# KwonGihyun/TweedieMix

Measured on AMD Instinct MI355X. Metric: denoise steps/sec @ SDXL 1024^2 K=3 concepts (fusion phase); images/sec at 1/2/4/8 GPUs, higher is better.
Workload: dtype bf16

## Files before the change

tweediemix_amd/csrc/norm_misc.hip:

```cpp
#include "common.h"

namespace {

typedef __attribute__((ext_vector_type(8))) __bf16 frag_ab;

__device__ __forceinline__ void unpack8(const uint4& v, float (&f)[8]) {
    f[0] = bf2f((bf16_t)(v.x & 0xffff)); f[1] = bf2f((bf16_t)(v.x >> 16));
    f[2] = bf2f((bf16_t)(v.y & 0xffff)); f[3] = bf2f((bf16_t)(v.y >> 16));
    f[4] = bf2f((bf16_t)(v.z & 0xffff)); f[5] = bf2f((bf16_t)(v.z >> 16));
    f[6] = bf2f((bf16_t)(v.w & 0xffff)); f[7] = bf2f((bf16_t)(v.w >> 16));
}
__device__ __forceinline__ uint4 pack8(const float (&f)[8]) {
    uint4 v;
    v.x = pack_bf2(f[0], f[1]); v.y = pack_bf2(f[2], f[3]); v.z = pack_bf2(f[4], f[5]); v.w = pack_bf2(f[6], f[7]);
    return v;
}

constexpr int GN_MAX_C = 4096;

#ifndef GN_T
#define GN_T 128
#endif
#ifndef GN_APPLY_U
#define GN_APPLY_U 2
#endif
#ifndef GN_APPLY_ITEMS
#define GN_APPLY_ITEMS 1024
#endif
#ifndef GN_APPLY_MAXB
#define GN_APPLY_MAXB 4096
#endif
__host__ __device__ inline int gn_chunks(int64_t HW) {
    int64_t c = HW / 8;
    if (c > GN_T) c = GN_T;
    if (c < 1) c = 1;
    return (int)c;
}

__global__ void __launch_bounds__(256) gn_stats_kernel(const bf16_t* __restrict__ X1, int C1, const bf16_t* __restrict__ X2, int C2,
                                                       float* __restrict__ ws, int64_t HW, int groups, int chunks,
                                                       unsigned long long* prof) {
    __shared__ float s_sum[GN_MAX_C], s_sq[GN_MAX_C];
    if (prof && threadIdx.x == 0) prof_enter(prof, (blockIdx.x | blockIdx.y) == 0, 0);
    const int C = C1 + C2, nvec = C >> 3, cpg = C / groups;
    const int b = blockIdx.y, ch = blockIdx.x, tid = threadIdx.x;
    const int64_t ppc = (HW + chunks - 1) / chunks;
    const int64_t p0 = (int64_t)ch * ppc;
    int64_t p1 = p0 + ppc; if (p1 > HW) p1 = HW;
    const int plane = nvec <= 256 ? 256 / nvec : 1;
    for (int v0 = 0; v0 < nvec; v0 += 256) {
        const int v = v0 + (nvec <= 256 ? tid % nvec : tid);
        const int pl = nvec <= 256 ? tid / nvec : 0;
        if (v < nvec && pl < plane) {
            float a[8] = {0, 0, 0, 0, 0, 0, 0, 0}, q[8] = {0, 0, 0, 0, 0, 0, 0, 0};
            const int c0 = v * 8;
            const bf16_t* src; int cs, cl;
            if (c0 < C1) { src = X1 + (int64_t)b * HW * C1; cs = C1; cl = c0; }
            else         { src = X2 + (int64_t)b * HW * C2; cs = C2; cl = c0 - C1; }
            int64_t p = p0 + pl;
            for (; p + 3 * plane < p1; p += 4 * plane) {
                uint4 raw[4];
#pragma unroll
                for (int u = 0; u < 4; ++u) raw[u] = *(const uint4*)(src + (p + u * plane) * cs + cl);
#pragma unroll
                for (int u = 0; u < 4; ++u) {
                    float f[8]; unpack8(raw[u], f);
#pragma unroll
                    for (int j = 0; j < 8; ++j) { a[j] += f[j]; q[j] += f[j] * f[j]; }
                }
            }
            for (; p < p1; p += plane) {
                const uint4 raw = *(const uint4*)(src + p * cs + cl);
                float f[8]; unpack8(raw, f);
#pragma unroll
                for (int j = 0; j < 8; ++j) { a[j] += f[j]; q[j] += f[j] * f[j]; }
            }
#pragma unroll
            for (int j = 0; j < 8; ++j) { s_sum[pl * C + c0 + j] = a[j]; s_sq[pl * C + c0 + j] = q[j]; }
        }
    }
    __syncthreads();
    if (tid < groups) {
        float s = 0.f, q = 0.f;
// ... 39 lines not shown
        s += (a0 + a1) + (a2 + a3); q += (b0 + b1) + (b2 + b3);
    }
    for (; blk < nblk; blk += J, row += step) { s += row[0]; q += row[Cs]; }
}
__global__ void __launch_bounds__(GN_CS_T) gn_finalize_cs_kernel(const float* __restrict__ cs1, int C1, const float* __restrict__ cs2, int C2,
                                                                 const float* __restrict__ gamma, const float* __restrict__ beta,
                                                                 float2* __restrict__ ss, int64_t HW, int groups, float eps,
                                                                 unsigned long long* prof) {
    __shared__ double s_red[2 * GN_CS_T / 64];
    __shared__ float s_ms[2];
    if (prof && threadIdx.x == 0) prof_enter(prof, (blockIdx.x | blockIdx.y) == 0, 0);
    const int C = C1 + C2, cpg = C / groups;
    const int g = blockIdx.x, b = blockIdx.y, tid = threadIdx.x;
    const int nblk = (int)(HW / 32);
    float gm = 0.f, bt = 0.f;
    if (tid < cpg) { gm = gamma[g * cpg + tid]; bt = beta[g * cpg + tid]; }
    const int c_lo = g * cpg, c_hi = c_lo + cpg;
    const int n1 = min(c_hi, C1) - min(c_lo, C1), n2 = cpg - n1;
    float s = 0.f, q = 0.f;
    gn_cs_walk(cs1 + (int64_t)b * nblk * 2 * C1 + c_lo, C1, n1, nblk, tid, s, q);
    if (n2 > 0) gn_cs_walk(cs2 + (int64_t)b * nblk * 2 * C2 + (max(c_lo, C1) - C1), C2, n2, nblk, tid, s, q);
    double sd = (double)s, qd = (double)q;
#pragma unroll
    for (int o = 32; o > 0; o >>= 1) { sd += __shfl_xor(sd, o); qd += __shfl_xor(qd, o); }
    if ((tid & 63) == 0) { s_red[(tid >> 6) * 2] = sd; s_red[(tid >> 6) * 2 + 1] = qd; }
    __syncthreads();
    if (tid == 0) {
        double st = 0.0, qt = 0.0;
#pragma unroll
        for (int w = 0; w < GN_CS_T / 64; ++w) { st += s_red[2 * w]; qt += s_red[2 * w + 1]; }
        const double n = (double)HW * cpg;
        const double mean = st / n;
        double var = qt / n - mean * mean; if (var < 0.0) var = 0.0;
        s_ms[0] = (float)mean; s_ms[1] = (float)(1.0 / sqrt(var + (double)eps));
    }
    __syncthreads();
    if (tid < cpg) {
        const float sc = s_ms[1] * gm;
        ss[(int64_t)b * C + c_lo + tid] = make_float2(sc, bt - s_ms[0] * sc);
    }
}

__device__ __forceinline__ float silu_fast(float x) {
    return x * __builtin_amdgcn_rcpf(1.0f + __builtin_amdgcn_exp2f(-1.4426950408889634f * x));
}

__device__ __forceinline__ float gn_quad_max(float x) {
    float y = __int_as_float(__builtin_amdgcn_update_dpp(0, __float_as_int(x), 0xB1, 0xf, 0xf, false));
    x = fmaxf(x, y);
    y = __int_as_float(__builtin_amdgcn_update_dpp(0, __float_as_int(x), 0x4E, 0xf, 0xf, false));
    return fmaxf(x, y);
}

template <int F8>
__global__ void __launch_bounds__(256) gn_apply_kernel(const bf16_t* __restrict__ X1, int C1, const bf16_t* __restrict__ X2, int C2,
                                                       bf16_t* __restrict__ Y, const float2* __restrict__ ss, int64_t HW, int silu,
                                                       unsigned long long* prof, unsigned char* __restrict__ Y8 = nullptr, unsigned char* __restrict__ S8 = nullptr) {
    __shared__ float2 s_ss[GN_MAX_C];
    const unsigned long long pt0 = (prof && threadIdx.x == 0) ? prof_now() : 0;
    const int C = C1 + C2, nvec = C >> 3;
    const int b = blockIdx.y, tid = threadIdx.x;
    for (int c = tid; c < C; c += 256) s_ss[c] = ss[(int64_t)b * C + c];
    __syncthreads();
    const int64_t total = HW * nvec;
    int64_t per = (total + gridDim.x - 1) / gridDim.x;
    if (F8) per = (per + 3) & ~(int64_t)3;
    const int64_t i0 = (int64_t)blockIdx.x * per;
    int64_t i1 = i0 + per; if (i1 > total) i1 = total;
    int64_t p = i0 / nvec; int v = (int)(i0 - p * nvec) + tid;
    while (v >= nvec) { v -= nvec; ++p; }
    const int step_p = 256 / nvec, step_v = 256 - step_p * nvec;
    constexpr int U = GN_APPLY_U;
    for (int64_t i = i0 + tid; i < i1; i += 256 * U) {
        uint4 raw[U]; int64_t pp[U]; int cc[U];
#pragma unroll
        for (int u = 0; u < U; ++u) {
            pp[u] = p; cc[u] = v * 8;
            if (i + u * 256 < i1) {
                const bf16_t* src = (cc[u] < C1) ? X1 + ((int64_t)b * HW + p) * C1 + cc[u] : X2 + ((int64_t)b * HW + p) * C2 + (cc[u] - C1);
                raw[u] = *(const uint4*)src;
            }
            p += step_p; v += step_v;
            if (v >= nvec) { v -= nvec; ++p; }
        }
#pragma unroll
        for (int u = 0; u < U; ++u) {
            if (i + u * 256 < i1) {
                float f[8]; unpack8(raw[u], f);
#pragma unroll
                for (int j = 0; j < 8; ++j) {
                    const float2 k = s_ss[cc[u] + j];
                    float y = f[j] * k.x + k.y;
                    if (silu) y = silu_fast(y);
                    f[j] = y;
                }
                if constexpr (F8) {
                    const uint4 pk = pack8(f);
                    unpack8(pk, f);
                    float am = 0.f;
#pragma unroll
                    for (int j = 0; j < 8; ++j) am = fmaxf(am, fabsf(f[j]));
                    am = gn_quad_max(am);
                    const int e = e8m0_for_amax(am);
                    const float inv = exp2_neg_int(e);
                    int q0 = __builtin_amdgcn_cvt_pk_fp8_f32(f[0] * inv, f[1] * inv, 0, false); q0 = __builtin_amdgcn_cvt_pk_fp8_f32(f[2] * inv, f[3] * inv, q0, true);
                    int q1 = __builtin_amdgcn_cvt_pk_fp8_f32(f[4] * inv, f[5] * inv, 0, false); q1 = __builtin_amdgcn_cvt_pk_fp8_f32(f[6] * inv, f[7] * inv, q1, true);
                    const int64_t row = (int64_t)b * HW + pp[u];
                    *(uint2*)(Y8 + row * C + cc[u]) = make_uint2((unsigned)q0, (unsigned)q1);
                    if ((tid & 3) == 0) S8[row * (C >> 5) + (cc[u] >> 5)] = (unsigned char)(e + 127);
                } else
                *(uint4*)(Y + ((int64_t)b * HW + pp[u]) * C + cc[u]) = pack8(f);
            }
        }
    }
    if (prof && threadIdx.x == 0) prof_leave(prof, 0, pt0, pt0, pt0);
}

constexpr int GN_SMALL_MAX_CW = 256, GN_SMALL_MAX_ELEMS = 65536;
__global__ void __launch_bounds__(256) gn_small_kernel(const bf16_t* __restrict__ X1, int C1, const bf16_t* __restrict__ X2, int C2, bf16_t* __restrict__ Y,
                                                       const float* __restrict__ gamma, const float* __restrict__ beta, int HW, int groups, int gpw, float eps, int silu,
                                                       unsigned long long* prof) {
    __shared__ float r_s[2048], r_q[2048];
    __shared__ double c_s[GN_SMALL_MAX_CW], c_q[GN_SMALL_MAX_CW];
    __shared__ float g_ms[16];
    __shared__ float2 s_ss[GN_SMALL_MAX_CW];
    const unsigned long long pt0 = (prof && threadIdx.x == 0) ? prof_enter(prof, (blockIdx.x | blockIdx.y) == 0, 0) : 0;
    const int C = C1 + C2, cpg = C / groups, cw = gpw * cpg, nv = cw >> 3, rs = 256 / nv;
    const int b = blockIdx.y, c0 = blockIdx.x * cw, tid = threadIdx.x;
    const int v = tid % nv, slot = tid / nv;
    const bool active = slot < rs;
    const int cg = c0 + v * 8;
    const bf16_t* src; int ld;
    if (cg < C1) { src = X1 + (int64_t)b * HW * C1 + cg; ld = C1; } else { src = X2 + (int64_t)b * HW * C2 + (cg - C1); ld = C2; }
    float s[8], q[8];
#pragma unroll
    for (int j = 0; j < 8; ++j) { s[j] = 0.f; q[j] = 0.f; }
    if (active) {
        int row = slot;
        for (; row + 3 * rs < HW; row += 4 * rs) {
            uint4 raw[4];
#pragma unroll
            for (int u = 0; u < 4; ++u) raw[u] = *(const uint4*)(src + (int64_t)(row + u * rs) * ld);
#pragma unroll
            for (int u = 0; u < 4; ++u) {
                float f[8]; unpack8(raw[u], f);
#pragma unroll
                for (int j = 0; j < 8; ++j) { s[j] += f[j]; q[j] += f[j] * f[j]; }
            }
        }
        for (; row < HW; row += rs) {
            float f[8]; unpack8(*(const uint4*)(src + (int64_t)row * ld), f);
#pragma unroll
            for (int j = 0; j < 8; ++j) { s[j] += f[j]; q[j] += f[j] * f[j]; }
        }
#pragma unroll
        for (int j = 0; j < 8; ++j) { r_s[slot * cw + v * 8 + j] = s[j]; r_q[slot * cw + v * 8 + j] = q[j]; }
    }
    __syncthreads();
    if (tid < cw) {
        double a = 0.0, d = 0.0;
        for (int k = 0; k < rs; ++k) { a += (double)r_s[k * cw + tid]; d += (double)r_q[k * cw + tid]; }
        c_s[tid] = a; c_q[tid] = d;
    }
    __syncthreads();
    if (tid < gpw) {
        double a = 0.0, d = 0.0;
        for (int k = 0; k < cpg; ++k) { a += c_s[tid * cpg + k]; d += c_q[tid * cpg + k]; }
        const double n = (double)HW * cpg, mean = a / n;
// ... 177 lines not shown
                                                           const int* __restrict__ secs, int nsec, int Mtot, int mrow0) {
    const int lane = threadIdx.x & 63;
    const int n = blockIdx.x * 4 + (threadIdx.x >> 6);
    if (n >= N) return;
    float acc[MAXM];
#pragma unroll
    for (int m = 0; m < MAXM; ++m) acc[m] = 0.f;
    const int nvec = K >> 3;
    for (int v = lane; v < nvec; v += 64) {
        const uint4 raw = *(const uint4*)(W + (int64_t)n * K + v * 8);
        float wf[8]; unpack8(raw, wf);
#pragma unroll
        for (int m = 0; m < MAXM; ++m) {
            if (m < M) {
                const float4 x0 = *(const float4*)(in + (int64_t)m * K + v * 8);
                const float4 x1 = *(const float4*)(in + (int64_t)m * K + v * 8 + 4);
                float xf[8] = {x0.x, x0.y, x0.z, x0.w, x1.x, x1.y, x1.z, x1.w};
                if (act_in) {
#pragma unroll
                    for (int j = 0; j < 8; ++j) xf[j] = silu_f(xf[j]);
                }
#pragma unroll
                for (int j = 0; j < 8; ++j) acc[m] += xf[j] * wf[j];
            }
        }
    }
#pragma unroll
    for (int m = 0; m < MAXM; ++m) {
#pragma unroll
        for (int o = 32; o > 0; o >>= 1) acc[m] += __shfl_xor(acc[m], o);
    }
    if (lane == 0) {
        int64_t base = 0; int ldn = N, col = n;
        if (secs) {
            int sidx = 0;
            while (sidx + 1 < nsec && secs[sidx + 1] <= n) ++sidx;
            base = (int64_t)secs[sidx] * Mtot; ldn = secs[sidx + 1] - secs[sidx]; col = n - secs[sidx];
        }
        for (int m = 0; m < M; ++m) {
            float y = acc[m] + (bias ? bias[n] : 0.f) + (add ? add[(int64_t)m * N + n] : 0.f);
            if (act_out) y = silu_f(y);
            out[base + (int64_t)(secs ? mrow0 + m : m) * ldn + col] = y;
        }
    }
}

struct PreMap { float w[16]; float b[4]; int on; };

template <int CIN>
__global__ void __launch_bounds__(256) conv_in_kernel(const float* __restrict__ x, const float* __restrict__ w,
                                                      const float* __restrict__ bias, bf16_t* __restrict__ y,
                                                      int B, int H, int W, int Cout, const PreMap pm) {
    extern __shared__ __attribute__((aligned(16))) float s_w[];
    constexpr int KK = 9 * CIN;
    const int tid = threadIdx.x, lane = tid & 63;
    const int q = __builtin_amdgcn_readfirstlane(tid >> 6);
    for (int i = tid; i < Cout * KK / 4; i += 256) ((float4*)s_w)[i] = ((const float4*)w)[i];
    __syncthreads();
    const int64_t npix = (int64_t)B * H * W;
    for (int64_t tile = blockIdx.x; tile * 64 < npix; tile += gridDim.x) {
    int64_t pix = tile * 64 + lane;
    const bool live = pix < npix;
    if (!live) pix = npix - 1;
    const int b = (int)(pix / ((int64_t)H * W)); const int rem = (int)(pix - (int64_t)b * H * W);
    const int oy = rem / W, ox = rem - oy * W;
    float patch[KK];
#pragma unroll
    for (int ky = 0; ky < 3; ++ky)
#pragma unroll
        for (int kx = 0; kx < 3; ++kx) {
            const int iy = oy + ky - 1, ix = ox + kx - 1;
            const bool ok = iy >= 0 && iy < H && ix >= 0 && ix < W;
            float v[CIN];
#pragma unroll
            for (int ci = 0; ci < CIN; ++ci) v[ci] = ok ? x[(((int64_t)b * CIN + ci) * H + iy) * W + ix] : 0.f;
            if (pm.on && CIN == 4) {
                float u[4];
#pragma unroll
                for (int co = 0; co < 4; ++co)
                    u[co] = ok ? pm.b[co] + pm.w[co * 4 + 0] * v[0] + pm.w[co * 4 + 1] * v[1] + pm.w[co * 4 + 2] * v[2] + pm.w[co * 4 + 3] * v[3] : 0.f;
#pragma unroll
                for (int co = 0; co < 4; ++co) v[co] = u[co];
            }
#pragma unroll
            for (int ci = 0; ci < CIN; ++ci) patch[(ky * 3 + kx) * CIN + ci] = v[ci];
        }
    const int cpq = Cout / 4;
    for (int c0 = q * cpq; c0 < (q + 1) * cpq; c0 += 8) {
        float o[8];
#pragma unroll 2
        for (int j = 0; j < 8; ++j) {
            const float* wr = s_w + (c0 + j) * KK;
            float a = bias ? bias[c0 + j] : 0.f;
#pragma unroll
            for (int k = 0; k < KK; ++k) a += patch[k] * wr[k];
            o[j] = a;
        }
        if (live) *(uint4*)(y + pix * Cout + c0) = pack8(o);
    }
    }
}

__global__ void __launch_bounds__(256) conv_out_kernel(const bf16_t* __restrict__ x, const bf16_t* __restrict__ w,
                                                       const float* __restrict__ bias, float* __restrict__ y,
                                                       int B, int H, int W, int Cin, int Cout) {
    const int lane = threadIdx.x & 63, fr = lane & 15, fg = lane >> 4;
    const int64_t npix = (int64_t)B * H * W;
    const int64_t pbase = ((int64_t)blockIdx.x * 4 + (threadIdx.x >> 6)) * 16;
    if (pbase >= npix) return;
    int64_t pix = pbase + fr; if (pix > npix - 1) pix = npix - 1;
    const int b = (int)(pix / ((int64_t)H * W)); const int rem = (int)(pix - (int64_t)b * H * W);
    const int oy = rem / W, ox = rem - oy * W;
    const int co = fr < Cout ? fr : Cout - 1;
    const bf16_t* wrow = w + (int64_t)co * 9 * Cin;
    f32x4 acc = {0.f, 0.f, 0.f, 0.f};
    const frag_ab zero = {0, 0, 0, 0, 0, 0, 0, 0};
    for (int tap = 0; tap < 9; ++tap) {
        const int ky = tap / 3, kx = tap - ky * 3;
        const int iy = oy + ky - 1, ix = ox + kx - 1;
        const bool ok = iy >= 0 && iy < H && ix >= 0 && ix < W;
        const bf16_t* src = x + (((int64_t)b * H + (ok ? iy : 0)) * W + (ok ? ix : 0)) * Cin;
        for (int c = 0; c < Cin; c += 32) {
            frag_ab a = *(const frag_ab*)(src + c + fg * 8);
            if (!ok) a = zero;
            const frag_ab wf = *(const frag_ab*)(wrow + tap * Cin + c + fg * 8);
            acc = __builtin_amdgcn_mfma_f32_16x16x32_bf16(a, wf, acc, 0, 0, 0);
        }
    }
    if (fr < Cout) {
        const float bv = bias ? bias[fr] : 0.f;
#pragma unroll
        for (int r = 0; r < 4; ++r) {
            const int64_t pp = pbase + fg * 4 + r;
            if (pp < npix) {
                const int bb = (int)(pp / ((int64_t)H * W)); const int64_t rr = pp - (int64_t)bb * H * W;
                y[((int64_t)bb * Cout + fr) * H * W + rr] = acc[r] + bv;
            }
        }
    }
}

}

extern "C" int tmix_groupnorm_ws_chunks(int64_t HW) { return gn_chunks(HW); }
extern "C" int64_t tmix_groupnorm_ws_floats(int B, int C, int groups) { return (int64_t)B * GN_T * groups * 2 + (int64_t)B * C * 2; }

extern "C" int tmix_groupnorm_nhwc_launches(int64_t HW, int C, int groups) {
    if (HW <= 0 || C <= 0 || groups <= 0 || (C % groups)) return 0;
    return gn_small_gpw(HW, C, groups) ? 1 : 3;
}

extern "C" int tmix_groupnorm_nhwc(const void* X1, int C1, const void* X2, int C2, void* Y, const float* gamma,
                                   const float* beta, float* ws, int B, int64_t HW, int groups, float eps, int silu,
                                   void* stream) {
    if (!X1 || !Y || !gamma || !beta || !ws) TMIX_FAIL(TMIX_EINVAL, "groupnorm: null pointer");
    if (C2 > 0 && !X2) TMIX_FAIL(TMIX_EINVAL, "groupnorm: C2 > 0 but X2 is null");
    const int C = C1 + C2;
    if (B <= 0 || HW <= 0 || C <= 0) TMIX_FAIL(TMIX_ESHAPE, "groupnorm: empty problem");
    if ((C1 % 8) || (C2 % 8) || C > GN_MAX_C || groups <= 0 || groups > 64 || (C % groups)) TMIX_FAIL(TMIX_ESHAPE, "groupnorm: C1=%d C2=%d groups=%d unsupported", C1, C2, groups);
    if (!aligned16(X1) || (X2 && !aligned16(X2)) || !aligned16(Y)) TMIX_FAIL(TMIX_EALIGN, "groupnorm: pointers must be 16-byte aligned");
    const int chunks = gn_chunks(HW);
    hipStream_t st = (hipStream_t)stream;
    unsigned long long* prof = tmix_prof_take();
    if (const int gpw = gn_small_gpw(HW, C, groups)) {
        gn_small_kernel<<<dim3(groups / gpw, B), 256, 0, st>>>((const bf16_t*)X1, C1, (const bf16_t*)X2, C2, (bf16_t*)Y, gamma, beta, (int)HW, groups, gpw, eps, silu, prof);
        TMIX_LAUNCH_CHECK();
        return TMIX_OK;
    }
    gn_stats_kernel<<<dim3(chunks, B), 256, 0, st>>>((const bf16_t*)X1, C1, (const bf16_t*)X2, C2, ws, HW, groups, chunks, prof);
    TMIX_LAUNCH_CHECK();
    float2* ss = (float2*)(ws + (int64_t)B * GN_T * groups * 2);
    gn_finalize_kernel<<<dim3(groups, B), 64, 0, st>>>(ws, gamma, beta, ss, C, HW, groups, chunks, eps);
    TMIX_LAUNCH_CHECK();
    int64_t nb = (HW * (C / 8) + GN_APPLY_ITEMS - 1) / GN_APPLY_ITEMS; if (nb < 1) nb = 1; if (nb > GN_APPLY_MAXB) nb = GN_APPLY_MAXB;
    gn_apply_kernel<0><<<dim3((unsigned)nb, B), 256, 0, st>>>((const bf16_t*)X1, C1, (const bf16_t*)X2, C2, (bf16_t*)Y, ss, HW, silu, prof);
    TMIX_LAUNCH_CHECK();
    return TMIX_OK;
}

static int gn_pre_entry(const void* X1, int C1, const void* X2, int C2, void* Y, void* S8, const float* gamma,
                        const float* beta, float* ws, int B, int64_t HW, int groups, float eps, int silu,
                        const float* cs1, int cs1_channels, const float* cs2, int cs2_channels, void* stream) {
    if (!X1 || !Y || !gamma || !beta || !ws || !cs1) TMIX_FAIL(TMIX_EINVAL, "groupnorm_pre: null pointer");
    if (S8 && ((C1 + C2) % 32)) TMIX_FAIL(TMIX_ESHAPE, "groupnorm_pre_f8: C must be a multiple of 32 (MX blocks)");
    if (C2 > 0 && !X2) TMIX_FAIL(TMIX_EINVAL, "groupnorm_pre: C2 > 0 but X2 is null");
    const int C = C1 + C2;
    if (cs1_channels <= 0 || cs2_channels < 0 || cs1_channels + cs2_channels != C || (cs2_channels > 0 && !cs2))
        TMIX_FAIL(TMIX_EINVAL, "groupnorm_pre: the partials cover %d + %d channels, the tensor has %d", cs1_channels, cs2_channels, C);
    if (B <= 0 || HW <= 0 || C <= 0) TMIX_FAIL(TMIX_ESHAPE, "groupnorm_pre: empty problem");
    if ((C1 % 8) || (C2 % 8) || C > GN_MAX_C || groups <= 0 || groups > 64 || (C % groups) || C / groups > 256) TMIX_FAIL(TMIX_ESHAPE, "groupnorm_pre: C1=%d C2=%d groups=%d unsupported", C1, C2, groups);
    if (HW % TMIX_COLSTATS_ROWS) TMIX_FAIL(TMIX_ESHAPE, "groupnorm_pre: HW=%lld must be a multiple of %d (the producers' partials cover 32-row blocks)", (long long)HW, TMIX_COLSTATS_ROWS);
    if (!aligned16(X1) || (X2 && !aligned16(X2)) || !aligned16(Y)) TMIX_FAIL(TMIX_EALIGN, "groupnorm_pre: pointers must be 16-byte aligned");
    hipStream_t st = (hipStream_t)stream;
    unsigned long long* prof = tmix_prof_take();
    float2* ss = (float2*)(ws + (int64_t)B * GN_T * groups * 2);
    gn_finalize_cs_kernel<<<dim3(groups, B), GN_CS_T, 0, st>>>(cs1, cs1_channels, cs2, cs2_channels, gamma, beta, ss, HW, groups, eps, prof);
    TMIX_LAUNCH_CHECK();
    int64_t nb = (HW * (C / 8) + GN_APPLY_ITEMS - 1) / GN_APPLY_ITEMS; if (nb < 1) nb = 1; if (nb > GN_APPLY_MAXB) nb = GN_APPLY_MAXB;
    if (S8) gn_apply_kernel<1><<<dim3((unsigned)nb, B), 256, 0, st>>>((const bf16_t*)X1, C1, (const bf16_t*)X2, C2, nullptr, ss, HW, silu, prof, (unsigned char*)Y, (unsigned char*)S8);
    else gn_apply_kernel<0><<<dim3((unsigned)nb, B), 256, 0, st>>>((const bf16_t*)X1, C1, (const bf16_t*)X2, C2, (bf16_t*)Y, ss, HW, silu, prof);
    TMIX_LAUNCH_CHECK();
    return TMIX_OK;
}

extern "C" int tmix_groupnorm_nhwc_pre(const void* X1, int C1, const void* X2, int C2, void* Y, const float* gamma,
                                       const float* beta, float* ws, int B, int64_t HW, int groups, float eps, int silu,
                                       const float* cs1, int cs1_channels, const float* cs2, int cs2_channels, void* stream) {
    return gn_pre_entry(X1, C1, X2, C2, Y, nullptr, gamma, beta, ws, B, HW, groups, eps, silu, cs1, cs1_channels, cs2, cs2_channels, stream);
}

extern "C" int tmix_groupnorm_nhwc_pre_f8(const void* X1, int C1, const void* X2, int C2, void* Y8, void* scales, const float* gamma,
                                          const float* beta, float* ws, int B, int64_t HW, int groups, float eps, int silu,
                                          const float* cs1, int cs1_channels, const float* cs2, int cs2_channels, void* stream) {
    if (!scales) TMIX_FAIL(TMIX_EINVAL, "groupnorm_pre_f8: null scale array");
    return gn_pre_entry(X1, C1, X2, C2, Y8, scales, gamma, beta, ws, B, HW, groups, eps, silu, cs1, cs1_channels, cs2, cs2_channels, stream);
}

extern "C" int tmix_layernorm(const void* X, void* Y, const float* gamma, const float* beta, int64_t rows, int C,
                              float eps, void* stream) {
    if (!X || !Y || !gamma || !beta) TMIX_FAIL(TMIX_EINVAL, "layernorm: null pointer");
    if (rows <= 0 || C <= 0) TMIX_FAIL(TMIX_ESHAPE, "layernorm: empty problem");
    if ((C % 8) || C > 2048) TMIX_FAIL(TMIX_ESHAPE, "layernorm: C=%d must be a multiple of 8 and <= 2048", C);
    if (!aligned16(X) || !aligned16(Y) || !aligned16(gamma) || !aligned16(beta)) TMIX_FAIL(TMIX_EALIGN, "layernorm: pointers must be 16-byte aligned");
    layernorm_kernel<<<(unsigned)((rows + 3) / 4), 256, 0, (hipStream_t)stream>>>((const bf16_t*)X, (bf16_t*)Y, gamma, beta, rows, C, eps);
    TMIX_LAUNCH_CHECK();
    return TMIX_OK;
}

__global__ void __launch_bounds__(256) quantize_fp8_rows_kernel(const bf16_t* __restrict__ X, int64_t ld, unsigned char* __restrict__ Q, int64_t ldq,
                                                                unsigned char* __restrict__ scale, int64_t rows, int K) {
    const int lane = threadIdx.x & 63;
    const int64_t r = (int64_t)blockIdx.x * 4 + (threadIdx.x >> 6);
    if (r >= rows) return;
    constexpr int MAXV = 16;
    const int nv = K >> 3;
    uint4 v[MAXV];
    float amax = 0.f;
#pragma unroll
    for (int u = 0; u < MAXV; ++u) {
        const int c = u * 64 + lane;
        if (c < nv) {
            v[u] = *(const uint4*)(X + r * ld + (int64_t)c * 8);
            const unsigned w[4] = {v[u].x, v[u].y, v[u].z, v[u].w};
#pragma unroll
            for (int k = 0; k < 4; ++k) amax = fmaxf(amax, fmaxf(fabsf(__uint_as_float(w[k] << 16)), fabsf(__uint_as_float(w[k] & 0xffff0000u))));
        }
    }
#pragma unroll
    for (int off = 32; off >= 1; off >>= 1) amax = fmaxf(amax, __shfl_xor(amax, off));
    const int e = e8m0_for_amax(amax);
    const float inv = exp2_neg_int(e);
    if (lane == 0) scale[r] = (unsigned char)(e + 127);
#pragma unroll
// ... 247 lines not shown
    if (count <= 0 || dim <= 0 || (dim & 1)) TMIX_FAIL(TMIX_ESHAPE, "timestep_embedding: count=%d dim=%d", count, dim);
    const int n = count * (dim / 2);
    timestep_embedding_kernel<<<(n + 255) / 256, 256, 0, (hipStream_t)stream>>>(values, out, count, dim);
    TMIX_LAUNCH_CHECK();
    return TMIX_OK;
}

static int linear_small_launch(const float* in, const void* W, const float* bias, const float* add, float* out, int M, int N, int K,
                               int act_in, int act_out, const int* secs, int nsec, hipStream_t st) {
    for (int m0 = 0; m0 < M; m0 += 16) {
        const int m = M - m0 < 16 ? M - m0 : 16;
        const float* in_c = in + (int64_t)m0 * K;
        const float* add_c = add ? add + (int64_t)m0 * N : nullptr;
        float* out_c = secs ? out : out + (int64_t)m0 * N;
        if (m <= 4) linear_small_kernel<4><<<(N + 3) / 4, 256, 0, st>>>(in_c, (const bf16_t*)W, bias, add_c, out_c, m, N, K, act_in, act_out, secs, nsec, M, m0);
        else        linear_small_kernel<16><<<(N + 3) / 4, 256, 0, st>>>(in_c, (const bf16_t*)W, bias, add_c, out_c, m, N, K, act_in, act_out, secs, nsec, M, m0);
        TMIX_LAUNCH_CHECK();
    }
    return TMIX_OK;
}

extern "C" int tmix_linear_small(const float* in, const void* W, const float* bias, const float* add, float* out,
                                 int M, int N, int K, int act_in, int act_out, void* stream) {
    if (!in || !W || !out) TMIX_FAIL(TMIX_EINVAL, "linear_small: null pointer");
    if (M <= 0 || M > 256 || N <= 0 || K <= 0 || (K % 8)) TMIX_FAIL(TMIX_ESHAPE, "linear_small: M=%d (1..256) N=%d K=%d (K %% 8 == 0)", M, N, K);
    if (!aligned16(in) || !aligned16(W)) TMIX_FAIL(TMIX_EALIGN, "linear_small: in/W must be 16-byte aligned");
    return linear_small_launch(in, W, bias, add, out, M, N, K, act_in, act_out, nullptr, 0, (hipStream_t)stream);
}

extern "C" int tmix_linear_small_sections(const float* in, const void* W, const float* bias, float* out, int M, int N, int K,
                                          int act_in, const int* sec_starts, int nsec, void* stream) {
    if (!in || !W || !out || !sec_starts) TMIX_FAIL(TMIX_EINVAL, "linear_small_sections: null pointer");
    if (M <= 0 || M > 256 || N <= 0 || K <= 0 || (K % 8) || nsec < 1) TMIX_FAIL(TMIX_ESHAPE, "linear_small_sections: M=%d (1..256) N=%d K=%d (K %% 8 == 0) nsec=%d", M, N, K, nsec);
    if (!aligned16(in) || !aligned16(W)) TMIX_FAIL(TMIX_EALIGN, "linear_small_sections: in/W must be 16-byte aligned");
    return linear_small_launch(in, W, bias, nullptr, out, M, N, K, act_in, 0, sec_starts, nsec, (hipStream_t)stream);
}

extern "C" int tmix_conv_in(const float* x_nchw, const float* w_ohwi, const float* bias, void* y_nhwc,
                            int B, int Cin, int H, int W, int Cout, void* stream) {
    return tmix_conv_in_pre(x_nchw, w_ohwi, bias, y_nhwc, B, Cin, H, W, Cout, nullptr, nullptr, stream);
}

extern "C" int tmix_conv_in_pre(const float* x_nchw, const float* w_ohwi, const float* bias, void* y_nhwc,
                                int B, int Cin, int H, int W, int Cout, const float* pre_w, const float* pre_b, void* stream) {
    if (!x_nchw || !w_ohwi || !y_nhwc) TMIX_FAIL(TMIX_EINVAL, "conv_in: null pointer");
    if (B <= 0 || H <= 0 || W <= 0 || Cout <= 0) TMIX_FAIL(TMIX_ESHAPE, "conv_in: bad shape");
    if (!aligned16(y_nhwc)) TMIX_FAIL(TMIX_EALIGN, "conv_in: output must be 16-byte aligned");
    if (Cout % 32) TMIX_FAIL(TMIX_ESHAPE, "conv_in: Cout=%d must be a multiple of 32", Cout);
    if (Cin != 3 && Cin != 4 && Cin != 8) TMIX_FAIL(TMIX_ESHAPE, "conv_in: Cin=%d (3: RGB image, 4: image latent, 8: video latent + image-latent features)", Cin);
    if (Cin != 4 && pre_w) TMIX_FAIL(TMIX_EINVAL, "conv_in: the latent pre-map is defined for 4 channels");
    if ((Cout * 9 * Cin) % 4) TMIX_FAIL(TMIX_ESHAPE, "conv_in: Cout*9*Cin must be a multiple of 4");
    if (!aligned16(w_ohwi)) TMIX_FAIL(TMIX_EALIGN, "conv_in: weights must be 16-byte aligned");
    const int64_t npix = (int64_t)B * H * W;
    const int64_t ntiles = (npix + 63) / 64;
    const int smem = Cout * 9 * Cin * 4;
    const int per_cu = smem > 80 * 1024 ? 1 : (smem > 52 * 1024 ? 2 : 3);
    const unsigned nb = (unsigned)(ntiles < 256 * per_cu ? ntiles : 256 * per_cu);
    if (smem > 150 * 1024) TMIX_FAIL(TMIX_ESHAPE, "conv_in: Cout=%d too large for the LDS weight stage", Cout);
    static int attr_smem[3] = {0, 0, 0};
    const int slot = Cin == 8 ? 2 : (Cin == 4 ? 1 : 0);
    if (smem > 64 * 1024 && smem > attr_smem[slot]) {
        hipError_t e = Cin == 8 ? hipFuncSetAttribute((const void*)conv_in_kernel<8>, hipFuncAttributeMaxDynamicSharedMemorySize, smem)
                     : Cin == 4 ? hipFuncSetAttribute((const void*)conv_in_kernel<4>, hipFuncAttributeMaxDynamicSharedMemorySize, smem)
                                : hipFuncSetAttribute((const void*)conv_in_kernel<3>, hipFuncAttributeMaxDynamicSharedMemorySize, smem);
        if (e != hipSuccess) TMIX_FAIL((int)e, "hipFuncSetAttribute: %s", hipGetErrorString(e));
        attr_smem[slot] = smem;
    }
    PreMap pm = {};
    if (pre_w) {
        pm.on = 1;
        for (int i = 0; i < 16; ++i) pm.w[i] = pre_w[i];
        for (int i = 0; i < 4; ++i) pm.b[i] = pre_b ? pre_b[i] : 0.f;
    }
    hipStream_t st = (hipStream_t)stream;
    if (Cin == 8) conv_in_kernel<8><<<nb, 256, smem, st>>>(x_nchw, w_ohwi, bias, (bf16_t*)y_nhwc, B, H, W, Cout, pm);
    else if (Cin == 3) conv_in_kernel<3><<<nb, 256, smem, st>>>(x_nchw, w_ohwi, bias, (bf16_t*)y_nhwc, B, H, W, Cout, pm);
    else          conv_in_kernel<4><<<nb, 256, smem, st>>>(x_nchw, w_ohwi, bias, (bf16_t*)y_nhwc, B, H, W, Cout, pm);
    TMIX_LAUNCH_CHECK();
    return TMIX_OK;
}

extern "C" int tmix_conv_out(const void* x_nhwc, const void* w_ohwi, const float* bias, float* y_nchw,
                             int B, int Cin, int H, int W, int Cout, void* stream) {
    if (!x_nhwc || !w_ohwi || !y_nchw) TMIX_FAIL(TMIX_EINVAL, "conv_out: null pointer");
    if (B <= 0 || H <= 0 || W <= 0 || Cout <= 0 || Cout > 16 || (Cin % 32)) TMIX_FAIL(TMIX_ESHAPE, "conv_out: Cin=%d (%%32) Cout=%d (<=16)", Cin, Cout);
    if (!aligned16(x_nhwc) || !aligned16(w_ohwi)) TMIX_FAIL(TMIX_EALIGN, "conv_out: pointers must be 16-byte aligned");
    const int64_t npix = (int64_t)B * H * W;
    const unsigned nb = (unsigned)((npix + 63) / 64);
    conv_out_kernel<<<nb, 256, 0, (hipStream_t)stream>>>((const bf16_t*)x_nhwc, (const bf16_t*)w_ohwi, bias, y_nchw, B, H, W, Cin, Cout);
    TMIX_LAUNCH_CHECK();
    return TMIX_OK;
}
```

Measured before the change: 32.99.

## Retile GroupNorm apply, move conv_in to MFMA, pipeline conv_out with LDS weights

GroupNorm apply now gives each thread a fixed 8-channel column and walks rows, so it holds per-channel scale/shift in registers and no longer stages them through LDS or does div/mod index arithmetic. Loads for the next rows are prefetched. conv_in is rewritten as fp32 MFMA 16x16x4 over 128-pixel tiles with a re-laid-out LDS weight stage. conv_out becomes persistent, stages weights in LDS when they fit, chunks channels and double-buffers its input fragments. Several kernels change at once, and conv_in/conv_out are a small share of a UNet step.

```diff
diff --git a/tweediemix_amd/csrc/norm_misc.hip b/tweediemix_amd/csrc/norm_misc.hip
--- a/tweediemix_amd/csrc/norm_misc.hip
+++ b/tweediemix_amd/csrc/norm_misc.hip
@@ -23,12 +23,6 @@
 #endif
 #ifndef GN_APPLY_U
 #define GN_APPLY_U 2
-#endif
-#ifndef GN_APPLY_ITEMS
-#define GN_APPLY_ITEMS 1024
-#endif
-#ifndef GN_APPLY_MAXB
-#define GN_APPLY_MAXB 4096
 #endif
 __host__ __device__ inline int gn_chunks(int64_t HW) {
     int64_t c = HW / 8;
@@ -174,45 +168,58 @@
     return fmaxf(x, y);
 }
 
+constexpr int GN_APPLY_T = 320;
+struct GnApplyGeom { int w, rows, ntile, ppw, shares; };
+static GnApplyGeom gn_apply_geom(int64_t HW, int C, bool f8) {
+    GnApplyGeom g;
+    const int nvec = C >> 3;
+    g.w = 1;
+    for (int d = 1; d <= 64 && d <= nvec; ++d)
+        if (nvec % d == 0 && (!f8 || d % 4 == 0)) g.w = d;
+    g.rows = GN_APPLY_T / g.w;
+    g.ntile = nvec / g.w;
+    const int64_t batch = (int64_t)g.rows * GN_APPLY_U;
+    int64_t shares = (HW + batch - 1) / batch;
+    const int64_t cap = 1024 / g.ntile > 1 ? 1024 / g.ntile : 1;
+    if (shares > cap) shares = cap;
+    g.ppw = (int)((HW + shares - 1) / shares);
+    g.shares = (int)((HW + g.ppw - 1) / g.ppw);
+    return g;
+}
+
 template <int F8>
-__global__ void __launch_bounds__(256) gn_apply_kernel(const bf16_t* __restrict__ X1, int C1, const bf16_t* __restrict__ X2, int C2,
-                                                       bf16_t* __restrict__ Y, const float2* __restrict__ ss, int64_t HW, int silu,
-                                                       unsigned long long* prof, unsigned char* __restrict__ Y8 = nullptr, unsigned char* __restrict__ S8 = nullptr) {
-    __shared__ float2 s_ss[GN_MAX_C];
+__global__ void __launch_bounds__(GN_APPLY_T) gn_apply_kernel(const bf16_t* __restrict__ X1, int C1, const bf16_t* __restrict__ X2, int C2,
+                                                              bf16_t* __restrict__ Y, const float2* __restrict__ ss, int64_t HW, int silu,
+                                                              int w, int ntile, int ppw,
+                                                              unsigned long long* prof, unsigned char* __restrict__ Y8 = nullptr, unsigned char* __restrict__ S8 = nullptr) {
     const unsigned long long pt0 = (prof && threadIdx.x == 0) ? prof_now() : 0;
-    const int C = C1 + C2, nvec = C >> 3;
+    const int C = C1 + C2;
     const int b = blockIdx.y, tid = threadIdx.x;
-    for (int c = tid; c < C; c += 256) s_ss[c] = ss[(int64_t)b * C + c];
-    __syncthreads();
-    const int64_t total = HW * nvec;
-    int64_t per = (total + gridDim.x - 1) / gridDim.x;
-    if (F8) per = (per + 3) & ~(int64_t)3;
-    const int64_t i0 = (int64_t)blockIdx.x * per;
-    int64_t i1 = i0 + per; if (i1 > total) i1 = total;
-    int64_t p = i0 / nvec; int v = (int)(i0 - p * nvec) + tid;
-    while (v >= nvec) { v -= nvec; ++p; }
-    const int step_p = 256 / nvec, step_v = 256 - step_p * nvec;
+    const int share = blockIdx.x / ntile, tile = blockIdx.x - share * ntile;
+    const int r = tid / w, rows = blockDim.x / w;
+    const int cc = (tile * w + (tid - r * w)) * 8;
+    const bf16_t* src; int64_t ld;
+    if (cc < C1) { src = X1 + (int64_t)b * HW * C1 + cc; ld = C1; } else { src = X2 + (int64_t)b * HW * C2 + (cc - C1); ld = C2; }
+    const int64_t p0 = (int64_t)share * ppw;
+    int64_t p1 = p0 + ppw; if (p1 > HW) p1 = HW;
     constexpr int U = GN_APPLY_U;
-    for (int64_t i = i0 + tid; i < i1; i += 256 * U) {
-        uint4 raw[U]; int64_t pp[U]; int cc[U];
+    int64_t p = p0 + r;
+    uint4 raw[U];
+#pragma unroll
+    for (int u = 0; u < U; ++u)
+        if (p + u * rows < p1) raw[u] = *(const uint4*)(src + (p + u * rows) * ld);
+    float2 k[8];
+#pragma unroll
+    for (int j = 0; j < 8; ++j) k[j] = ss[(int64_t)b * C + cc + j];
+    while (p < p1) {
 #pragma unroll
         for (int u = 0; u < U; ++u) {
-            pp[u] = p; cc[u] = v * 8;
-            if (i + u * 256 < i1) {
-                const bf16_t* src = (cc[u] < C1) ? X1 + ((int64_t)b * HW + p) * C1 + cc[u] : X2 + ((int64_t)b * HW + p) * C2 + (cc[u] - C1);
-                raw[u] = *(const uint4*)src;
-            }
-            p += step_p; v += step_v;
-            if (v >= nvec) { v -= nvec; ++p; }
-        }
-#pragma unroll
-        for (int u = 0; u < U; ++u) {
-            if (i + u * 256 < i1) {
+            const int64_t pp = p + u * rows;
+            if (pp < p1) {
                 float f[8]; unpack8(raw[u], f);
 #pragma unroll
                 for (int j = 0; j < 8; ++j) {
-                    const float2 k = s_ss[cc[u] + j];
-                    float y = f[j] * k.x + k.y;
+                    float y = f[j] * k[j].x + k[j].y;
                     if (silu) y = silu_fast(y);
                     f[j] = y;
                 }
@@ -227,15 +234,26 @@
                     const float inv = exp2_neg_int(e);
                     int q0 = __builtin_amdgcn_cvt_pk_fp8_f32(f[0] * inv, f[1] * inv, 0, false); q0 = __builtin_amdgcn_cvt_pk_fp8_f32(f[2] * inv, f[3] * inv, q0, true);
                     int q1 = __builtin_amdgcn_cvt_pk_fp8_f32(f[4] * inv, f[5] * inv, 0, false); q1 = __builtin_amdgcn_cvt_pk_fp8_f32(f[6] * inv, f[7] * inv, q1, true);
-                    const int64_t row = (int64_t)b * HW + pp[u];
-                    *(uint2*)(Y8 + row * C + cc[u]) = make_uint2((unsigned)q0, (unsigned)q1);
-                    if ((tid & 3) == 0) S8[row * (C >> 5) + (cc[u] >> 5)] = (unsigned char)(e + 127);
+                    const int64_t row = (int64_t)b * HW + pp;
+                    *(uint2*)(Y8 + row * C + cc) = make_uint2((unsigned)q0, (unsigned)q1);
+                    if ((tid & 3) == 0) S8[row * (C >> 5) + (cc >> 5)] = (unsigned char)(e + 127);
                 } else
-                *(uint4*)(Y + ((int64_t)b * HW + pp[u]) * C + cc[u]) = pack8(f);
-            }
-        }
+                *(uint4*)(Y + ((int64_t)b * HW + pp) * C + cc) = pack8(f);
+            }
+        }
+        p += (int64_t)U * rows;
+#pragma unroll
+        for (int u = 0; u < U; ++u)
+            if (p + u * rows < p1) raw[u] = *(const uint4*)(src + (p + u * rows) * ld);
     }
     if (prof && threadIdx.x == 0) prof_leave(prof, 0, pt0, pt0, pt0);
+}
+static void gn_apply_launch(bool f8, const bf16_t* X1, int C1, const bf16_t* X2, int C2, void* Y, void* S8, const float2* ss, int B, int64_t HW, int silu,
+                            unsigned long long* prof, hipStream_t st) {
+    const GnApplyGeom g = gn_apply_geom(HW, C1 + C2, f8);
+    const dim3 grid((unsigned)(g.shares * g.ntile), B);
+    if (f8) gn_apply_kernel<1><<<grid, g.rows * g.w, 0, st>>>(X1, C1, X2, C2, nullptr, ss, HW, silu, g.w, g.ntile, g.ppw, prof, (unsigned char*)Y, (unsigned char*)S8);
+    else gn_apply_kernel<0><<<grid, g.rows * g.w, 0, st>>>(X1, C1, X2, C2, (bf16_t*)Y, ss, HW, silu, g.w, g.ntile, g.ppw, prof);
 }
 
 constexpr int GN_SMALL_MAX_CW = 256, GN_SMALL_MAX_ELEMS = 65536;
@@ -519,89 +537,168 @@
                                                       const float* __restrict__ bias, bf16_t* __restrict__ y,
                                                       int B, int H, int W, int Cout, const PreMap pm) {
     extern __shared__ __attribute__((aligned(16))) float s_w[];
-    constexpr int KK = 9 * CIN;
-    const int tid = threadIdx.x, lane = tid & 63;
-    const int q = __builtin_amdgcn_readfirstlane(tid >> 6);
-    for (int i = tid; i < Cout * KK / 4; i += 256) ((float4*)s_w)[i] = ((const float4*)w)[i];
-    __syncthreads();
-    const int64_t npix = (int64_t)B * H * W;
-    for (int64_t tile = blockIdx.x; tile * 64 < npix; tile += gridDim.x) {
-    int64_t pix = tile * 64 + lane;
-    const bool live = pix < npix;
-    if (!live) pix = npix - 1;
-    const int b = (int)(pix / ((int64_t)H * W)); const int rem = (int)(pix - (int64_t)b * H * W);
-    const int oy = rem / W, ox = rem - oy * W;
-    float patch[KK];
-#pragma unroll
-    for (int ky = 0; ky < 3; ++ky)
-#pragma unroll
-        for (int kx = 0; kx < 3; ++kx) {
-            const int iy = oy + ky - 1, ix = ox + kx - 1;
-            const bool ok = iy >= 0 && iy < H && ix >= 0 && ix < W;
-            float v[CIN];
-#pragma unroll
-            for (int ci = 0; ci < CIN; ++ci) v[ci] = ok ? x[(((int64_t)b * CIN + ci) * H + iy) * W + ix] : 0.f;
-            if (pm.on && CIN == 4) {
-                float u[4];
-#pragma unroll
-                for (int co = 0; co < 4; ++co)
-                    u[co] = ok ? pm.b[co] + pm.w[co * 4 + 0] * v[0] + pm.w[co * 4 + 1] * v[1] + pm.w[co * 4 + 2] * v[2] + pm.w[co * 4 + 3] * v[3] : 0.f;
-#pragma unroll
-                for (int co = 0; co < 4; ++co) v[co] = u[co];
-            }
-#pragma unroll
-            for (int ci = 0; ci < CIN; ++ci) patch[(ky * 3 + kx) * CIN + ci] = v[ci];
-        }
-    const int cpq = Cout / 4;
-    for (int c0 = q * cpq; c0 < (q + 1) * cpq; c0 += 8) {
-        float o[8];
-#pragma unroll 2
-        for (int j = 0; j < 8; ++j) {
-            const float* wr = s_w + (c0 + j) * KK;
-            float a = bias ? bias[c0 + j] : 0.f;
-#pragma unroll
-            for (int k = 0; k < KK; ++k) a += patch[k] * wr[k];
-            o[j] = a;
-        }
-        if (live) *(uint4*)(y + pix * Cout + c0) = pack8(o);
-    }
-    }
-}
-
+    __shared__ float s_pm[20];
+    constexpr int KS = (CIN + 3) / 4, KK = 9 * CIN;
+    const int tid = threadIdx.x, lane = tid & 63, fr = lane & 15, fg = lane >> 4;
+    const int nit = Cout * 9 * KS;
+    for (int i0 = 0; i0 < nit; i0 += 1024) {
+        float4 v[4]; int dst[4];
+#pragma unroll
+        for (int u = 0; u < 4; ++u) {
+            const int i = min(i0 + u * 256 + tid, nit - 1);
+            const int co = i / (9 * KS), t = i - co * 9 * KS, tap = t / KS, ks = t - tap * KS;
+            const int cl = co & 31;
+            dst[u] = (tap * KS + ks) * Cout + (co & ~31) + ((cl >> 2) & 1) * 16 + (cl >> 3) * 4 + (cl & 3);
+            const float* wr = w + (int64_t)co * KK + tap * CIN + ks * 4;
+            if constexpr (CIN % 4 == 0) v[u] = *(const float4*)wr;
+            else { v[u].x = wr[0]; v[u].y = ks * 4 + 1 < CIN ? wr[1] : 0.f; v[u].z = ks * 4 + 2 < CIN ? wr[2] : 0.f; v[u].w = 0.f; }
+        }
+#pragma unroll
+        for (int u = 0; u < 4; ++u) ((float4*)s_w)[dst[u]] = v[u];
+    }
+    if (tid < 16) s_pm[tid] = pm.w[tid]; else if (tid < 20) s_pm[tid] = pm.b[tid - 16];
+    __syncthreads();
+    const int64_t npix = (int64_t)B * H * W, HWp = (int64_t)H * W;
+    for (int64_t tile = blockIdx.x; tile * 128 < npix; tile += gridDim.x) {
+        const int64_t pbase = tile * 128 + (tid >> 6) * 32;
+        if (pbase >= npix) continue;
+        float pt[2][9 * KS];
+        const float* src[2][9]; bool ok[2][9];
+#pragma unroll
+        for (int px = 0; px < 2; ++px) {
+            int64_t pix = pbase + px * 16 + fr; if (pix > npix - 1) pix = npix - 1;
+            const int b = (int)(pix / HWp); const int rem = (int)(pix - (int64_t)b * HWp);
+            const int oy = rem / W, ox = rem - oy * W;
+#pragma unroll
+            for (int tap = 0; tap < 9; ++tap) {
+                const int iy = oy + tap / 3 - 1, ix = ox + tap % 3 - 1;
+                ok[px][tap] = iy >= 0 && iy < H && ix >= 0 && ix < W;
+                src[px][tap] = x + (int64_t)b * CIN * HWp + (ok[px][tap] ? (int64_t)iy * W + ix : 0);
+            }
+        }
+        if (CIN == 4 && pm.on) {
+            float v[2][9][4];
+#pragma unroll
+            for (int px = 0; px < 2; ++px)
+#pragma unroll
+                for (int tap = 0; tap < 9; ++tap)
+#pragma unroll
+                    for (int ci = 0; ci < 4; ++ci) v[px][tap][ci] = src[px][tap][ci * HWp];
+            const float m0 = s_pm[fg * 4 + 0], m1 = s_pm[fg * 4 + 1], m2 = s_pm[fg * 4 + 2], m3 = s_pm[fg * 4 + 3], mb = s_pm[16 + fg];
+#pragma unroll
+            for (int px = 0; px < 2; ++px)
+#pragma unroll
+                for (int tap = 0; tap < 9; ++tap) {
+                    const float u = mb + m0 * v[px][tap][0] + m1 * v[px][tap][1] + m2 * v[px][tap][2] + m3 * v[px][tap][3];
+                    pt[px][tap] = ok[px][tap] ? u : 0.f;
+                }
+        } else {
+#pragma unroll
+            for (int px = 0; px < 2; ++px)
+#pragma unroll
+                for (int tap = 0; tap < 9; ++tap)
+#pragma unroll
+                    for (int ks = 0; ks < KS; ++ks) {
+                        const int ci = ks * 4 + fg;
+                        const float v = src[px][tap][(ci < CIN ? ci : 0) * HWp];
+                        pt[px][tap * KS + ks] = (ok[px][tap] && ci < CIN) ? v : 0.f;
+                    }
+        }
+        for (int c0 = 0; c0 < Cout; c0 += 32) {
+            f32x4 acc[2][2];
+#pragma unroll
+            for (int h = 0; h < 2; ++h) {
+                f32x4 bv = {0.f, 0.f, 0.f, 0.f};
+                if (bias) { const float* bp = bias + c0 + fg * 8 + h * 4; bv = (f32x4){bp[0], bp[1], bp[2], bp[3]}; }
+                acc[0][h] = bv; acc[1][h] = bv;
+            }
+            const float* wp = s_w + ((int64_t)c0 + fr) * 4 + fg;
+#pragma unroll
+            for (int t = 0; t < 9 * KS; ++t) {
+                const float a0 = wp[t * Cout * 4], a1 = wp[t * Cout * 4 + 64];
+#pragma unroll
+                for (int px = 0; px < 2; ++px) {
+                    acc[px][0] = __builtin_amdgcn_mfma_f32_16x16x4f32(a0, pt[px][t], acc[px][0], 0, 0, 0);
+                    acc[px][1] = __builtin_amdgcn_mfma_f32_16x16x4f32(a1, pt[px][t], acc[px][1], 0, 0, 0);
+                }
+            }
+#pragma unroll
+            for (int px = 0; px < 2; ++px) {
+                const int64_t pix = pbase + px * 16 + fr;
+                const float o[8] = {acc[px][0][0], acc[px][0][1], acc[px][0][2], acc[px][0][3], acc[px][1][0], acc[px][1][1], acc[px][1][2], acc[px][1][3]};
+                if (pix < npix) *(uint4*)(y + pix * Cout + c0 + fg * 8) = pack8(o);
+            }
+        }
+    }
+}
+
+template <int WLDS, int CH>
 __global__ void __launch_bounds__(256) conv_out_kernel(const bf16_t* __restrict__ x, const bf16_t* __restrict__ w,
                                                        const float* __restrict__ bias, float* __restrict__ y,
                                                        int B, int H, int W, int Cin, int Cout) {
+    extern __shared__ __attribute__((aligned(16))) bf16_t s_wo[];
     const int lane = threadIdx.x & 63, fr = lane & 15, fg = lane >> 4;
-    const int64_t npix = (int64_t)B * H * W;
-    const int64_t pbase = ((int64_t)blockIdx.x * 4 + (threadIdx.x >> 6)) * 16;
-    if (pbase >= npix) return;
-    int64_t pix = pbase + fr; if (pix > npix - 1) pix = npix - 1;
-    const int b = (int)(pix / ((int64_t)H * W)); const int rem = (int)(pix - (int64_t)b * H * W);
-    const int oy = rem / W, ox = rem - oy * W;
+    const int KK = 9 * Cin, ldw = WLDS ? KK + 8 : KK;
+    if (WLDS) {
+        const int vpr = KK >> 3, nv = Cout * vpr;
+        for (int i0 = 0; i0 < nv; i0 += 6 * 256) {
+            uint4 v[6];
+#pragma unroll
+            for (int u = 0; u < 6; ++u) v[u] = *(const uint4*)(w + (int64_t)min(i0 + u * 256 + (int)threadIdx.x, nv - 1) * 8);
+#pragma unroll
+            for (int u = 0; u < 6; ++u) {
+                const int i = min(i0 + u * 256 + (int)threadIdx.x, nv - 1), ro = i / vpr;
+                *(uint4*)(s_wo + ro * ldw + (i - ro * vpr) * 8) = v[u];
+            }
+        }
+        __syncthreads();
+    }
     const int co = fr < Cout ? fr : Cout - 1;
-    const bf16_t* wrow = w + (int64_t)co * 9 * Cin;
-    f32x4 acc = {0.f, 0.f, 0.f, 0.f};
+    const bf16_t* wrow = (WLDS ? (const bf16_t*)s_wo : w) + (int64_t)co * ldw + fg * 8;
+    const int64_t npix = (int64_t)B * H * W, HWp = (int64_t)H * W;
+    const int nb = Cin / (32 * CH), nsteps = 9 * nb;
     const frag_ab zero = {0, 0, 0, 0, 0, 0, 0, 0};
-    for (int tap = 0; tap < 9; ++tap) {
-        const int ky = tap / 3, kx = tap - ky * 3;
-        const int iy = oy + ky - 1, ix = ox + kx - 1;
-        const bool ok = iy >= 0 && iy < H && ix >= 0 && ix < W;
-        const bf16_t* src = x + (((int64_t)b * H + (ok ? iy : 0)) * W + (ok ? ix : 0)) * Cin;
-        for (int c = 0; c < Cin; c += 32) {
-            frag_ab a = *(const frag_ab*)(src + c + fg * 8);
-            if (!ok) a = zero;
-            const frag_ab wf = *(const frag_ab*)(wrow + tap * Cin + c + fg * 8);
-            acc = __builtin_amdgcn_mfma_f32_16x16x32_bf16(a, wf, acc, 0, 0, 0);
-        }
-    }
-    if (fr < Cout) {
-        const float bv = bias ? bias[fr] : 0.f;
-#pragma unroll
-        for (int r = 0; r < 4; ++r) {
-            const int64_t pp = pbase + fg * 4 + r;
-            if (pp < npix) {
-                const int bb = (int)(pp / ((int64_t)H * W)); const int64_t rr = pp - (int64_t)bb * H * W;
-                y[((int64_t)bb * Cout + fr) * H * W + rr] = acc[r] + bv;
+    const float bv = (bias && fr < Cout) ? bias[fr] : 0.f;
+    for (int64_t pbase = ((int64_t)blockIdx.x * 4 + (threadIdx.x >> 6)) * 16; pbase < npix; pbase += (int64_t)gridDim.x * 64) {
+        int64_t pix = pbase + fr; if (pix > npix - 1) pix = npix - 1;
+        const int b = (int)(pix / HWp); const int rem = (int)(pix - (int64_t)b * HWp);
+        const int oy = rem / W, ox = rem - oy * W;
+        const bf16_t* xc = x + ((int64_t)b * HWp + rem) * Cin + fg * 8;
+        auto load_step = [&](int tap, int cb, frag_ab (&a)[CH]) {
+            const int ky = tap / 3, kx = tap - ky * 3;
+            const int iy = oy + ky - 1, ix = ox + kx - 1;
+            const bool ok = iy >= 0 && iy < H && ix >= 0 && ix < W;
+            const bf16_t* src = xc + (ok ? ((ky - 1) * W + (kx - 1)) * (int64_t)Cin : 0) + cb * 32 * CH;
+#pragma unroll
+            for (int j = 0; j < CH; ++j) {
+                const frag_ab v = *(const frag_ab*)(src + j * 32);
+                a[j] = ok ? v : zero;
+            }
+        };
+        f32x4 acc = {0.f, 0.f, 0.f, 0.f};
+        frag_ab cur[CH], nxt[CH];
+        load_step(0, 0, cur);
+        int tap = 0, cb = 0;
+        for (int s = 0; s < nsteps; ++s) {
+            int ntap = tap, ncb = cb + 1;
+            if (ncb == nb) { ncb = 0; ++ntap; }
+            if (ntap > 8) { ntap = 8; ncb = nb - 1; }
+            load_step(ntap, ncb, nxt);
+            const bf16_t* wp = wrow + tap * Cin + cb * 32 * CH;
+#pragma unroll
+            for (int j = 0; j < CH; ++j)
+                acc = __builtin_amdgcn_mfma_f32_16x16x32_bf16(cur[j], *(const frag_ab*)(wp + j * 32), acc, 0, 0, 0);
+#pragma unroll
+            for (int j = 0; j < CH; ++j) cur[j] = nxt[j];
+            tap = ntap; cb = ncb;
+        }
+        if (fr < Cout) {
+            const int64_t pp0 = pbase + fg * 4;
+            int bb = (int)(pp0 / HWp); int64_t rr = pp0 - (int64_t)bb * HWp;
+#pragma unroll
+            for (int r = 0; r < 4; ++r) {
+                if (pp0 + r < npix) y[((int64_t)bb * Cout + fr) * HWp + rr] = acc[r] + bv;
+                if (++rr == HWp) { rr = 0; ++bb; }
             }
         }
     }
@@ -639,8 +736,7 @@
     float2* ss = (float2*)(ws + (int64_t)B * GN_T * groups * 2);
     gn_finalize_kernel<<<dim3(groups, B), 64, 0, st>>>(ws, gamma, beta, ss, C, HW, groups, chunks, eps);
     TMIX_LAUNCH_CHECK();
-    int64_t nb = (HW * (C / 8) + GN_APPLY_ITEMS - 1) / GN_APPLY_ITEMS; if (nb < 1) nb = 1; if (nb > GN_APPLY_MAXB) nb = GN_APPLY_MAXB;
-    gn_apply_kernel<0><<<dim3((unsigned)nb, B), 256, 0, st>>>((const bf16_t*)X1, C1, (const bf16_t*)X2, C2, (bf16_t*)Y, ss, HW, silu, prof);
+    gn_apply_launch(false, (const bf16_t*)X1, C1, (const bf16_t*)X2, C2, Y, nullptr, ss, B, HW, silu, prof, st);
     TMIX_LAUNCH_CHECK();
     return TMIX_OK;
 }
@@ -663,9 +759,7 @@
     float2* ss = (float2*)(ws + (int64_t)B * GN_T * groups * 2);
     gn_finalize_cs_kernel<<<dim3(groups, B), GN_CS_T, 0, st>>>(cs1, cs1_channels, cs2, cs2_channels, gamma, beta, ss, HW, groups, eps, prof);
     TMIX_LAUNCH_CHECK();
-    int64_t nb = (HW * (C / 8) + GN_APPLY_ITEMS - 1) / GN_APPLY_ITEMS; if (nb < 1) nb = 1; if (nb > GN_APPLY_MAXB) nb = GN_APPLY_MAXB;
-    if (S8) gn_apply_kernel<1><<<dim3((unsigned)nb, B), 256, 0, st>>>((const bf16_t*)X1, C1, (const bf16_t*)X2, C2, nullptr, ss, HW, silu, prof, (unsigned char*)Y, (unsigned char*)S8);
-    else gn_apply_kernel<0><<<dim3((unsigned)nb, B), 256, 0, st>>>((const bf16_t*)X1, C1, (const bf16_t*)X2, C2, (bf16_t*)Y, ss, HW, silu, prof);
+    gn_apply_launch(S8 != nullptr, (const bf16_t*)X1, C1, (const bf16_t*)X2, C2, Y, S8, ss, B, HW, silu, prof, st);
     TMIX_LAUNCH_CHECK();
     return TMIX_OK;
 }
@@ -1019,8 +1113,8 @@
     if ((Cout * 9 * Cin) % 4) TMIX_FAIL(TMIX_ESHAPE, "conv_in: Cout*9*Cin must be a multiple of 4");
     if (!aligned16(w_ohwi)) TMIX_FAIL(TMIX_EALIGN, "conv_in: weights must be 16-byte aligned");
     const int64_t npix = (int64_t)B * H * W;
-    const int64_t ntiles = (npix + 63) / 64;
-    const int smem = Cout * 9 * Cin * 4;
+    const int64_t ntiles = (npix + 127) / 128;
+    const int smem = Cout * 9 * ((Cin + 3) / 4) * 16;
     const int per_cu = smem > 80 * 1024 ? 1 : (smem > 52 * 1024 ? 2 : 3);
     const unsigned nb = (unsigned)(ntiles < 256 * per_cu ? ntiles : 256 * per_cu);
     if (smem > 150 * 1024) TMIX_FAIL(TMIX_ESHAPE, "conv_in: Cout=%d too large for the LDS weight stage", Cout);
@@ -1053,8 +1147,16 @@
     if (B <= 0 || H <= 0 || W <= 0 || Cout <= 0 || Cout > 16 || (Cin % 32)) TMIX_FAIL(TMIX_ESHAPE, "conv_out: Cin=%d (%%32) Cout=%d (<=16)", Cin, Cout);
     if (!aligned16(x_nhwc) || !aligned16(w_ohwi)) TMIX_FAIL(TMIX_EALIGN, "conv_out: pointers must be 16-byte aligned");
     const int64_t npix = (int64_t)B * H * W;
-    const unsigned nb = (unsigned)((npix + 63) / 64);
-    conv_out_kernel<<<nb, 256, 0, (hipStream_t)stream>>>((const bf16_t*)x_nhwc, (const bf16_t*)w_ohwi, bias, y_nchw, B, H, W, Cin, Cout);
-    TMIX_LAUNCH_CHECK();
-    return TMIX_OK;
-}
+    const int64_t ntiles = (npix + 63) / 64;
+    const unsigned nb = (unsigned)(ntiles < 512 ? ntiles : 512);
+    const int smem = Cout * (9 * Cin + 8) * 2;
+    const int nch = Cin / 32, ch = nch % 5 == 0 ? 5 : (nch % 4 == 0 ? 4 : (nch % 3 == 0 ? 3 : (nch % 2 == 0 ? 2 : 1)));
+    const bool lds = smem <= 64 * 1024;
+#define CONV_OUT_GO(WL, CHN) conv_out_kernel<WL, CHN><<<nb, 256, WL ? smem : 0, (hipStream_t)stream>>>((const bf16_t*)x_nhwc, (const bf16_t*)w_ohwi, bias, y_nchw, B, H, W, Cin, Cout)
+#define CONV_OUT_CH(CHN) do { if (lds) CONV_OUT_GO(1, CHN); else CONV_OUT_GO(0, CHN); } while (0)
+    switch (ch) { case 5: CONV_OUT_CH(5); break; case 4: CONV_OUT_CH(4); break; case 3: CONV_OUT_CH(3); break; case 2: CONV_OUT_CH(2); break; default: CONV_OUT_CH(1); }
+#undef CONV_OUT_CH
+#undef CONV_OUT_GO
+    TMIX_LAUNCH_CHECK();
+    return TMIX_OK;
+}
```

New measurement: 33.18 (median of 6 runs). No clear change (+0.6%).
